# meteorologytoday/XLab-FFTBarotropic

Measured on AMD Instinct MI355X. Metric: RK4 steps/sec, 4096x4096 periodic grid, higher is better.
Workload: dtype f32; 1 GPU; 4096x4096 kuo2004 initial field, nu=6.5, L=600 km, dt=0.75 s, 4 RK stages/step, fused HIP path; parallelism=single

## Files before the change

xlab-fftbarotropic_amd/csrc/fb_col_full.h:

```cpp
#pragma once
#include "fb_kernels.h"

#define CF_THREADS 1024
#define CF_X1_CF 16384
#define CF_X2_STR 68
#define CF_X2_CF (16 * 16 * CF_X2_STR)
#define CF_GX_CF 2048
#define CF_LDS_CF (CF_X2_CF + 512 + CF_GX_CF)
#define CF_LDS_BYTES (CF_LDS_CF * 8)

struct FullArgs {
    const cf *Tin;
    const cf *Zbase;
    cf *Zcur, *Acc, *Zout;
    cf *W4;
    long fstride;
    int P;
    int ntiles;
    int ntiles_run;
    int nsub;
    int stage;
    float nu, dt;
    SpecCoef coef;
    const cf *tw256;
    const cf *tw4096;
    long sub_rows;
    float wscale;
};

FB_DEV void cf_xchg_waves(cf *lds, cf *v, int w, int lane)
{
#pragma unroll
    for (int r = 0; r < 16; ++r) lds_wr(&lds[(r * 16 + w) * 64 + lane], v[r]);
    lds_barrier();
#pragma unroll
    for (int r = 0; r < 16; ++r) v[r] = lds_rd(&lds[(w * 16 + r) * 64 + lane]);
    lds_barrier();
}

template <bool SYNC>
FB_DEV void cf_xchg_lanes(cf *lds, cf *v, int w, int l, int c)
{
    cf *reg = lds + w * (16 * CF_X2_STR);
#pragma unroll
    for (int r = 0; r < 16; ++r) lds_wr(&reg[r * CF_X2_STR + l * 4 + c], v[r]);
    __builtin_amdgcn_wave_barrier();
#pragma unroll
    for (int r = 0; r < 16; ++r) v[r] = lds_rd(&reg[l * CF_X2_STR + r * 4 + c]);
    if (SYNC) lds_barrier();
    else { asm volatile("s_waitcnt lgkmcnt(0)" ::: "memory"); __builtin_amdgcn_wave_barrier(); }
}

#define CF_FENCE() __builtin_amdgcn_sched_barrier(0)
FB_DEV cf cf_mul(cf a, cf b) { return cmul_split(a, b); }
FB_DEV cf cf_mulc(cf a, cf b) { return cmulc_split(a, b); }

template <int DIR> FB_DEV void cf_bfly16(cf *v)
{
    fft4<DIR>(v[0], v[4], v[8], v[12]);  CF_FENCE();
    fft4<DIR>(v[1], v[5], v[9], v[13]);  CF_FENCE();
    fft4<DIR>(v[2], v[6], v[10], v[14]); CF_FENCE();
    fft4<DIR>(v[3], v[7], v[11], v[15]); CF_FENCE();
    v[5]  = mul_w16<1, DIR, true>(v[5]);  v[6]  = mul_w16<2, DIR, true>(v[6]);  v[7]  = mul_w16<3, DIR, true>(v[7]);
    v[9]  = mul_w16<2, DIR, true>(v[9]);  v[10] = mul_w16<4, DIR, true>(v[10]); v[11] = mul_w16<6, DIR, true>(v[11]);
    v[13] = mul_w16<3, DIR, true>(v[13]); v[14] = mul_w16<6, DIR, true>(v[14]); v[15] = mul_w16<9, DIR, true>(v[15]);
    CF_FENCE();
    fft4<DIR>(v[0], v[1], v[2], v[3]);     CF_FENCE();
    fft4<DIR>(v[4], v[5], v[6], v[7]);     CF_FENCE();
    fft4<DIR>(v[8], v[9], v[10], v[11]);   CF_FENCE();
    fft4<DIR>(v[12], v[13], v[14], v[15]); CF_FENCE();
    cf t;
    t = v[1];  v[1]  = v[4];  v[4]  = t;
    t = v[2];  v[2]  = v[8];  v[8]  = t;
    t = v[3];  v[3]  = v[12]; v[12] = t;
    t = v[6];  v[6]  = v[9];  v[9]  = t;
    t = v[7];  v[7]  = v[13]; v[13] = t;
    t = v[11]; v[11] = v[14]; v[14] = t;
}

template <int DIR>
FB_DEV void cf_fft4096(cf *lds, const cf *tabA, const cf *tabB, cf (*v)[16], int w, int l, int c, int lane)
{
    if (DIR < 0) {
#pragma unroll
        for (int col = 0; col < 2; ++col) {
            cf_bfly16<-1>(v[col]);
#pragma unroll
            for (int k1 = 1; k1 < 16; ++k1) { v[col][k1] = cf_mul(v[col][k1], tabB[w * k1]); if ((k1 & 3) == 3) CF_FENCE(); }
            cf_xchg_waves(lds, v[col], w, lane);
            CF_FENCE();
        }
        const cf a = tabA[l * w];
#pragma unroll
        for (int col = 0; col < 2; ++col) {
            cf_bfly16<-1>(v[col]);
            v[col][0] = cf_mul(v[col][0], a);
#pragma unroll
            for (int k2 = 1; k2 < 16; ++k2) { v[col][k2] = cf_mul(v[col][k2], cf_mul(a, tabB[l * k2])); if ((k2 & 3) == 3) CF_FENCE(); }
            cf_xchg_lanes<false>(lds, v[col], w, l, c);
            CF_FENCE();
        }
#pragma unroll
        for (int col = 0; col < 2; ++col) { cf_bfly16<-1>(v[col]); CF_FENCE(); }
    } else {
#pragma unroll
        for (int col = 0; col < 2; ++col) {
            cf_bfly16<+1>(v[col]);
#pragma unroll
            for (int lr = 1; lr < 16; ++lr) { v[col][lr] = cf_mulc(v[col][lr], cf_mul(tabA[lr * w], tabB[lr * l])); if ((lr & 3) == 3) CF_FENCE(); }
            if (col == 0) cf_xchg_lanes<false>(lds, v[col], w, l, c);
            else cf_xchg_lanes<true>(lds, v[col], w, l, c);
            CF_FENCE();
        }
#pragma unroll
        for (int col = 0; col < 2; ++col) {
            cf_bfly16<+1>(v[col]);
#pragma unroll
            for (int wr = 1; wr < 16; ++wr) { v[col][wr] = cf_mulc(v[col][wr], tabB[wr * w]); if ((wr & 3) == 3) CF_FENCE(); }
            cf_xchg_waves(lds, v[col], w, lane);
            CF_FENCE();
        }
#pragma unroll
        for (int col = 0; col < 2; ++col) { cf_bfly16<+1>(v[col]); CF_FENCE(); }
    }
}

FB_DEV float4 cf_ld4(const void *ubase, unsigned voff) { return *reinterpret_cast<const float4 *>(static_cast<const char *>(ubase) + voff); }
FB_DEV void cf_st4(void *ubase, unsigned voff, float4 x) { *reinterpret_cast<float4 *>(static_cast<char *>(ubase) + voff) = x; }
FB_DEV void cf_st4_w4(void *ubase, unsigned voff, float4 x) { st4<true>(static_cast<char *>(ubase) + voff, x); }

template <int STAGE, int NSUB>
__global__ void __launch_bounds__(CF_THREADS) k_col_full(FullArgs a)
{
    extern __shared__ __attribute__((aligned(16))) unsigned char smem_raw[];
    cf *lds = reinterpret_cast<cf *>(smem_raw);
    cf *tabB = lds + CF_X2_CF, *tabA = tabB + 256;
    float *gxt = reinterpret_cast<float *>(tabA + 256);
    const int tid = threadIdx.x, lane = tid & 63, l = lane >> 2, c = lane & 3;
    const int w = __builtin_amdgcn_readfirstlane(tid >> 6);

    constexpr int nsub = NSUB;
    const int ntg = gridDim.x / nsub;
    const int k1 = NSUB == 1 ? 0 : blockIdx.x / ntg, bt = blockIdx.x - k1 * ntg;
    int tile = bt;
    if ((ntg & 7) == 0) tile = (bt & 7) * (ntg >> 3) + (bt >> 3);
    if (tile >= a.ntiles_run) return;

    const int ky0 = tile * 8 + 2 * c;
    const unsigned voff_m = (unsigned)((l * a.P + 2 * c) * (int)sizeof(cf));
    const size_t ubase_m = ((size_t)(k1 * a.sub_rows + 16 * w) * a.P + (size_t)tile * 8) * sizeof(cf);
    const size_t rstep = (size_t)256 * a.P * sizeof(cf);
    const unsigned voff_s = (unsigned)(lane * (int)sizeof(float4));
    const size_t ubase_s = ((((size_t)k1 * (a.ntiles + 1) + tile) * 16) * CF_THREADS + (size_t)w * 64) * sizeof(float4);
    const size_t sstep = (size_t)CF_THREADS * sizeof(float4);

    constexpr bool PRIME = STAGE == 4;
    cf v[2][16];
    {
        const char *src = reinterpret_cast<const char *>(a.Tin) + ubase_m;
        float4 tin[16];
        if (!PRIME) {
#pragma unroll
            for (int i = 0; i < 16; ++i) tin[i] = ld4<true>(src + i * rstep + voff_m);
        }
        float g4[4];
#pragma unroll
        for (int i = 0; i < 4; ++i) g4[i] = a.coef.gx[nsub * (tid + i * CF_THREADS) + k1];
        if (tid < 256) { tabB[tid] = a.tw256[tid]; tabA[tid] = a.tw4096[tid]; }
#pragma unroll
        for (int i = 0; i < 4; ++i) {
            const int ik = tid + i * CF_THREADS;
            gxt[((ik >> 4) & 15) + 16 * (ik & 15) + (ik & ~255)] = g4[i];
        }
        if (!PRIME) {
#pragma unroll
            for (int i = 0; i < 16; ++i) { v[0][i] = cf_make(tin[i].x, tin[i].y); v[1][i] = cf_make(tin[i].z, tin[i].w); }
        }
    }
    __syncthreads();
    if (!PRIME) cf_fft4096<-1>(lds, tabA, tabB, v, w, l, c, lane);

    const char *Z0 = reinterpret_cast<const char *>(a.Zbase) + ubase_s;
    char *ZC = reinterpret_cast<char *>(a.Zcur) + ubase_s, *AC = reinterpret_cast<char *>(a.Acc) + ubase_s,
         *ZO = reinterpret_cast<char *>(a.Zout) + ubase_s;
    const float gya = a.coef.gy[ky0], gyb = a.coef.gy[ky0 + 1];
    auto ky2_of = [](float g) { asm volatile("" : "+v"(g)); return (double)g * (double)g; };
    constexpr bool PRIME_ = STAGE == 4;
    const bool pada = PRIME_ && ky0 >= a.coef.hy, padb = PRIME_ && ky0 + 1 >= a.coef.hy;
    constexpr int stage = STAGE;
    const float nu = a.nu, dt = a.dt, hdt = (stage == 2) ? a.dt : a.dt / 2.0f;
    constexpr int DEPTH = STAGE == 0 ? 2 : 1;
#ifndef CF_REMAKE_ZC
#define CF_REMAKE_ZC 1
#endif
    constexpr bool REMAKE_ZC = CF_REMAKE_ZC && STAGE == 1;
    float4 q0[DEPTH], q1[DEPTH], q2[DEPTH];
    auto load_k3 = [&](int k3) {
        const int sl = k3 % DEPTH;
        q0[sl] = ld4<false>(Z0 + k3 * sstep + voff_s);
        if (stage != 0) q2[sl] = ld4<true>(AC + k3 * sstep + voff_s);
        if (stage != 0 && !REMAKE_ZC) q1[sl] = ld4<false>(ZC + k3 * sstep + voff_s);
    };
    if (!PRIME) {
#pragma unroll
        for (int k3 = 0; k3 < DEPTH; ++k3) load_k3(k3);
    }
#pragma unroll
    for (int k3 = 0; k3 < (PRIME ? 0 : 16); ++k3) {
        const int sl = k3 % DEPTH;
        const int ik2 = w + 256 * k3 + 16 * l, ikx = nsub * ik2 + k1;
        const float gx = gxt[l + 16 * w + 256 * k3];
        const double kx2 = (double)gx * (double)gx;
        const float lapa = (float)(-(kx2 + ky2_of(gya))), lapb = (float)(-(kx2 + ky2_of(gyb)));
        const float mska = coef_mask(a.coef, ikx, ky0), mskb = coef_mask(a.coef, ikx, ky0 + 1);
        const float4 z0 = q0[sl];
        float4 zc = z0;
        if (REMAKE_ZC) {
            const float4 ac = q2[sl];
            zc = make_float4(__builtin_fmaf(ac.x, hdt, z0.x), __builtin_fmaf(ac.y, hdt, z0.y), __builtin_fmaf(ac.z, hdt, z0.z), __builtin_fmaf(ac.w, hdt, z0.w));
        } else if (stage != 0) zc = q1[sl];
        float4 k;
        k.x = (v[0][k3].x + (zc.x * lapa) * nu) * mska; k.y = (v[0][k3].y + (zc.y * lapa) * nu) * mska;
        k.z = (v[1][k3].x + (zc.z * lapb) * nu) * mskb; k.w = (v[1][k3].y + (zc.w * lapb) * nu) * mskb;
        float4 acc, zn;
        if (stage == 0) {
            acc = k;
            zn = make_float4(__builtin_fmaf(k.x, hdt, z0.x), __builtin_fmaf(k.y, hdt, z0.y), __builtin_fmaf(k.z, hdt, z0.z), __builtin_fmaf(k.w, hdt, z0.w));
        } else if (stage < 3) {
            const float4 ac = q2[sl];
            acc = make_float4(ac.x + 2.0f * k.x, ac.y + 2.0f * k.y, ac.z + 2.0f * k.z, ac.w + 2.0f * k.w);
            zn = make_float4(z0.x + k.x * hdt, z0.y + k.y * hdt, z0.z + k.z * hdt, z0.w + k.w * hdt);
        } else {
            const float4 ac = q2[sl];
            acc = ac;
            zn = make_float4(z0.x + (ac.x + k.x) * dt / 6.0f, z0.y + (ac.y + k.y) * dt / 6.0f,
                             z0.z + (ac.z + k.z) * dt / 6.0f, z0.w + (ac.w + k.w) * dt / 6.0f);
        }
        v[0][k3] = cf_make(zn.x, zn.y); v[1][k3] = cf_make(zn.z, zn.w);
        if (k3 + DEPTH < 16) load_k3(k3 + DEPTH);
        if (stage < 3) { st4<true>(AC + k3 * sstep + voff_s, acc); cf_st4(ZC + k3 * sstep, voff_s, zn); }
        else cf_st4(ZO + k3 * sstep, voff_s, zn);
        CF_FENCE();
    }

    const char *ZN = PRIME ? Z0 : (stage < 3 ? ZC : ZO);
#pragma unroll 1
    for (int f = 0; f < 4; ++f) {
        if (f > 0 || PRIME) {
            const unsigned vs = (unsigned)launder((int)voff_s);
#pragma unroll
            for (int k3 = 0; k3 < 16; ++k3) {
                const float4 z = cf_ld4(ZN + k3 * sstep, vs);
                v[0][k3] = cf_make(z.x, z.y); v[1][k3] = cf_make(z.z, z.w);
            }
        }
        const bool psi = f >= 2, use_gx = (f == 0 || f == 3);
        const int lkx = launder(l);
#pragma unroll
        for (int k3 = 0; k3 < 16; ++k3) {
            cf za = v[0][k3], zb = v[1][k3];
            const float gx = gxt[16 * w + 256 * k3 + lkx];
            if (psi) {
                const double kx2 = (double)gx * (double)gx;
                const float lia = (nsub * (w + 256 * k3 + 16 * l) + k1 == 0 && ky0 == 0) ? 1.0f : (float)(-(kx2 + ky2_of(gya)));
                const float lib = (float)(-(kx2 + ky2_of(gyb)));
                za = pada ? cf_make(0.f, 0.f) : cf_make(za.x / lia, za.y / lia);
                zb = padb ? cf_make(0.f, 0.f) : cf_make(zb.x / lib, zb.y / lib);
            }
            const float ka = (use_gx ? gx : gya) * a.wscale, kb = (use_gx ? gx : gyb) * a.wscale;
            v[0][k3] = cf_make(-za.y * ka, za.x * ka);
            v[1][k3] = cf_make(-zb.y * kb, zb.x * kb);
            CF_FENCE();
        }
        cf_fft4096<+1>(lds, tabA, tabB, v, w, l, c, lane);
        char *dst = reinterpret_cast<char *>(a.W4) + (size_t)f * a.fstride * sizeof(cf) + ubase_m;
        const unsigned vm = (unsigned)launder((int)voff_m);
#pragma unroll
        for (int i = 0; i < 16; ++i)
            cf_st4_w4(dst + i * rstep, vm, make_float4(v[0][i].x, v[0][i].y, v[1][i].x, v[1][i].y));
    }
}

template <bool TO_FULL>
__global__ void __launch_bounds__(256) k_full_relayout(const cf *__restrict__ in, cf *__restrict__ out, int P, int N1, int N2, int ntiles, int nsub, int hy)
{
    const size_t total = (size_t)nsub * (ntiles + 1) * 16 * CF_THREADS * 2;
    for (size_t idx = (size_t)blockIdx.x * blockDim.x + threadIdx.x; idx < total; idx += (size_t)gridDim.x * blockDim.x) {
        const int col = (int)(idx & 1);
        const int tid = (int)((idx >> 1) & (CF_THREADS - 1));
        const int k3 = (int)((idx >> 11) & 15);
        const int st = (int)(idx >> 15);
        const int k1 = st / (ntiles + 1), tile = st - k1 * (ntiles + 1);
        const int w = tid >> 6, l = (tid >> 2) & 15, c = tid & 3;
        const int kx = nsub * (w + 16 * l + 256 * k3) + k1, ky = tile * 8 + 2 * c + col;
        const int cc = kx % N1, d = kx / N1;
        const size_t p3 = (size_t)(N2 * cc + d) * P + ky;
        if (ky >= hy) { if (TO_FULL) out[idx] = cf_make(0.f, 0.f); continue; }
        if (TO_FULL) out[idx] = in[p3]; else out[p3] = in[idx];
    }
}
```

xlab-fftbarotropic_amd/csrc/fftbaro.hip:

```cpp
#include <hip/hip_runtime.h>
#include <algorithm>
#include <cmath>
#include <cstdio>
#include <cstdlib>
#include <cstring>
#include <mutex>
#include <set>
#include <string>
#include <type_traits>
#include <utility>
#include <vector>

#include "../../include/fftbaro.h"
#include "fb_kernels.h"
#include "fb_keff.h"
#include "fb_azim.h"
#include "fb_spectra.h"
#include "fb_tracer.h"
#include "fb_particles.h"
#include "fb_tangent.h"
#include "fb_adjoint.h"
#include "fb_col_full.h"
#include "fb_row3.h"
#include "fb_row8.h"
// ... 724 lines not shown
        finish_groups(c);
        return FB_OK;
    }
    const size_t maxe = (size_t)c->nx * (P0 + 16 * (NC - 1));
    const int nbuf = xp != XP_COLS ? 9 : 1;
    cf *buf = nullptr;
    if (hipMalloc((void **)&buf, maxe * nbuf * sizeof(cf)) != hipSuccess) { hipGetLastError(); return FB_OK; }
    hipMemsetAsync(buf, 0, maxe * nbuf * sizeof(cf), c->stream);
    hipEvent_t e0, e1;
    hipEventCreate(&e0); hipEventCreate(&e1);
    auto probe = [&](int P) -> int {
        ColGroup G = c->grp[0]; G.ncols = P;
        if (xp == XP_COLS) return launch_col_strided<+1>(c, G, buf, 1, 0);
        FullArgs a; memset(&a, 0, sizeof(a));
        a.Tin = buf; a.W4 = buf + maxe; a.Zbase = buf + 5 * maxe; a.Zcur = buf + 6 * maxe; a.Acc = buf + 7 * maxe; a.Zout = buf + 8 * maxe;
        a.fstride = (long)c->nx * P; a.P = P; a.ntiles = (c->ny / 2) / 8;
        a.ntiles_run = a.ntiles; a.nsub = xp; a.stage = 1; a.nu = 0.f; a.dt = 0.f; a.coef = make_coef(c); a.tw256 = c->d_tw_256;
        a.tw4096 = xp == XP_FULL1 ? c->d_tw_big : c->d_tw_4096; a.sub_rows = 4096;
        return launch_full(c, a);
    };
    const bool verbose = c->tune_verbose;
    hipEventRecord(e0, c->stream);
    for (int it = 0; it < 400; ++it) {
        if (probe(P0) != FB_OK) break;
        if ((it & 7) == 7) {
            hipEventRecord(e1, c->stream); hipEventSynchronize(e1);
            float ms = 0.f;
            if (hipEventElapsedTime(&ms, e0, e1) != hipSuccess || ms > 30.f) break;
        }
    }
    float tbest[8]; for (int k = 0; k < NC; ++k) tbest[k] = 1e30f;
    for (int rep = 0; rep < 6; ++rep)
        for (int k = 0; k < NC; ++k) {
            hipEventRecord(e0, c->stream);
            const int rc = probe(P0 + 16 * k);
            hipEventRecord(e1, c->stream);
            hipEventSynchronize(e1);
            float ms = 0.f;
            if (rc == FB_OK && hipEventElapsedTime(&ms, e0, e1) == hipSuccess && ms < tbest[k]) tbest[k] = ms;
        }
    float best = 1e30f; int bestP = P0;
    for (int k = 0; k < NC; ++k) {
        if (verbose) fprintf(stderr, "fftbaro: pitch probe P=%d %.4f ms\n", P0 + 16 * k, tbest[k]);
        if (tbest[k] < best * 0.99f) { best = tbest[k]; bestP = P0 + 16 * k; }
    }
    if (verbose) fprintf(stderr, "fftbaro: pitch %d -> %d\n", P0, bestP);
    c->P = c->KA = c->katot = c->grp[0].ncols = bestP;
    finish_groups(c);
    hipEventDestroy(e0); hipEventDestroy(e1);
    hipFree(buf);
    hipGetLastError();
    return FB_OK;
}

static int ensure_scratch(fb_ctx *c)
{
    if (!c->d_scratch) {
        hipError_t e = hipMalloc((void **)&c->d_scratch, priv_elems(c) * sizeof(cf));
        if (e != hipSuccess) return fail(FB_ENOMEM, "scratch allocation failed");
    }
    return FB_OK;
}

static unsigned magic_div(int d) { return d > 0 ? (unsigned)((1ull << 32) / (unsigned)d) + 1u : 0u; }
static RowView view_single(const fb_ctx *c, const cf *base, long fstride)
{
    RowView v; memset(&v, 0, sizeof(v));
    v.a = v.b = v.f = base; v.fstrA = v.fstrB = v.fstrF = fstride; v.ka = v.ka0 = c->P; v.kb = 0; v.kf = 16; v.katot = 0x7fffffff;
    return v;
}
static RowView view_slab(const fb_ctx *c, const cf *const *bufs, int nfields)
{
    RowView v; memset(&v, 0, sizeof(v));
    v.a = bufs[0]; v.b = c->nact > 1 ? bufs[1] : bufs[0]; v.f = c->KF > 0 ? bufs[c->nact] : bufs[0];
    v.ka = c->KA; v.ka0 = c->grp[0].ncols; v.kb = c->nact > 1 ? c->grp[1].ncols : 0; v.kf = c->KF > 0 ? c->KF : 16;
    v.katot = c->katot;
    v.fstrA = (long)c->XL * v.ka0; v.fstrB = (long)c->XL * v.kb; v.fstrF = (long)c->XL * v.kf;
    v.sstrA = (long)nfields * v.fstrA; v.sstrB = (long)nfields * v.fstrB; v.sstrF = (long)nfields * v.fstrF;
    v.magA = magic_div(v.ka); v.magF = magic_div(v.kf);
    return v;
}
static RowArgs row_args_base(const fb_ctx *c)
{
    RowArgs a; memset(&a, 0, sizeof(a));
    a.x0 = 0; a.nx = c->XL; a.tw_bwd = c->d_tw_row_bwd; a.tw_fwd = c->d_tw_row_fwd; a.t_frozen = 1;
    return a;
}

static int r2c_private(fb_ctx *c, const float *d_real, cf *dst)
{
    RowArgs a = row_args_base(c); a.rin = d_real; a.T = view_single(c, dst, 0);
    int rc;
    if ((rc = launch_row<ROW_FWD>(c, a))) return rc;
    if ((rc = launch_col_strided<-1>(c, c->grp[0], dst, 1, 0))) return rc;
    return launch_col_block<-1>(c, c->grp[0], dst, 1, 0);
}

static int c2r_private(fb_ctx *c, cf *work, float *d_real, float scale)
{
    int rc;
    if ((rc = launch_col_block<+1>(c, c->grp[0], work, 1, 0))) return rc;
    if ((rc = launch_col_strided<+1>(c, c->grp[0], work, 1, 0))) return rc;
    RowArgs a = row_args_base(c); a.M = view_single(c, work, 0); a.rout = d_real; a.scale = scale;
    return launch_row<ROW_INV>(c, a);
}

static bool state_tm(const fb_ctx *c) { return c->N2 >= 32; }
static int state_convert(fb_ctx *c, const ColGroup &G, const cf *in, cf *out, bool to_tm)
{
    if (G.ncols == 0) return FB_OK;
    if (!state_tm(c)) { HIPCHK(hipMemcpyAsync(out, in, grp_elems(c, G) * sizeof(cf), hipMemcpyDeviceToDevice, c->stream)); return FB_OK; }
    const size_t total = grp_elems(c, G);
    return launch_n(c, to_tm ? k_state_relayout<true> : k_state_relayout<false>, total, in, out, c->nx, G.ncols, c->N2);
}

static int relayout(fb_ctx *c, const cf *in, cf *out, bool to_private)
{
    const size_t total = priv_elems(c);
    return launch_n(c, to_private ? k_spec_relayout<true> : k_spec_relayout<false>, total, in, out, c->nx, c->hy, c->P, c->N1, c->N2);
}

extern "C" int fb_r2c(fb_ctx *c, const float *d_in, float *d_out)
{
    if (!c || !d_in || !d_out) return fail(FB_EINVAL, "fb_r2c: NULL");
    NEED_SINGLE(c);
    int rc;
    if ((rc = ensure_scratch(c))) return rc;
    HIPCHK(hipMemsetAsync(c->d_scratch, 0, priv_elems(c) * sizeof(cf), c->stream));
    if ((rc = r2c_private(c, d_in, c->d_scratch))) return rc;
    return relayout(c, c->d_scratch, (cf *)d_out, false);
}

extern "C" int fb_c2r(fb_ctx *c, const float *d_in, float *d_out, int normalize)
{
    if (!c || !d_in || !d_out) return fail(FB_EINVAL, "fb_c2r: NULL");
    NEED_SINGLE(c);
    int rc;
    if ((rc = ensure_scratch(c))) return rc;
    if ((rc = relayout(c, (const cf *)d_in, c->d_scratch, true))) return rc;
    const float scale = normalize ? 1.0f / (float)((size_t)c->nx * c->ny) : 1.0f;
    return c2r_private(c, c->d_scratch, d_out, scale);
}

struct GroupBufs { cf *ZA, *ZB, *ACC, *w4_send, *w4_recv, *t_send, *t_recv; };

struct Beside { cf *c0[3], *c1[3], *acc[3]; };

struct fb_model {
    fb_ctx *c;
    float nu, dt;
    GroupBufs gb[3];
    bool phase_flow;
    XPass xpass;
    bool prescale;
    bool use_graph, warmed;
    hipGraphExec_t graph_exec;
    const float *graph_src; hipStream_t graph_stream;
    float *src;
    int *src_nz;
    cf *rec_work[3], *rec_send[3];
    float *keff_fields;
    void *keff_red; size_t keff_red_cap;
    float *azim_fields;
    void *azim_red; size_t azim_red_cap;
    float *pres_ref;
    unsigned char rec_work_nf[3], rec_send_nf[3];
    void *spec_red;
    int primed;
    Beside tr;
    float kappa;
    bool tracer;
    double *pt; int pt_n;
    float *pt_uv;
    Beside tg[FB_TANGENTS_MAX];
    int tg_n;
    cf *tg_j[3];
    double *tg_red;
    cf *ad_tape; int ad_depth, ad_fill;
    Beside ad;
    float *ad_real;
    bool adjoint;
};

#include "fb_transport.h"
struct fb_slab {
    fb_ctx *c;
    fb_model *m;
    fb_transport tp;
    bool connected, owns_streams;
    hipStream_t comp, comm;
    hipEvent_t ev_f[4], ev_r[8], ev_w4, ev_t, ev_tg[2], ev_rows_done, ev_fwd_done, ev_misc[2];
    int nfg, nch;
    int ncg;
    int step_ops;
};
#include "fb_entry.h"

static int model_create_impl(fb_model **out, fb_ctx *c, float nu, float dt, bool phase_flow)
{
    if (!out || !c) return fail(FB_EINVAL, "fb_model_create: NULL");
    *out = nullptr;
    fb_model *m = new fb_model();
    memset(m, 0, sizeof(*m));
    m->c = c; m->nu = nu; m->dt = dt; m->phase_flow = phase_flow;
    m->xpass = phase_flow ? XP_COLS : choose_xpass(c);
    m->prescale = m->xpass != XP_COLS && c->world == 1 && c->row == RK_ROWQ && !c->no_prescale;
    int rc = FB_OK;
    auto alloc0 = [&](cf **p, size_t elems) {
        if (rc || elems == 0) return;
        if (hipMalloc((void **)p, elems * sizeof(cf)) != hipSuccess) { rc = fail(FB_ENOMEM, "model allocation failed"); return; }
        if (hipMemsetAsync(*p, 0, elems * sizeof(cf), c->stream) != hipSuccess) rc = fail(FB_EHIP, "hipMemsetAsync failed");
    };
    for (int g = 0; g < c->ngroups; ++g) {
        const size_t n = grp_elems(c, c->grp[g]);
        GroupBufs &B = m->gb[g];
        alloc0(&B.ZA, n);
        if (g < c->nact) { alloc0(&B.ZB, n); alloc0(&B.ACC, n); }
        alloc0(&B.w4_send, 4 * n); alloc0(&B.t_send, n);
        if (c->world > 1) { alloc0(&B.w4_recv, 4 * n); alloc0(&B.t_recv, n); }
        else { B.w4_recv = B.w4_send; B.t_recv = B.t_send; }
    }
    if (rc) { fb_model_destroy(m); return rc; }
    *out = m;
    return FB_OK;
}

extern "C" int fb_model_create(fb_model **out, fb_ctx *c, float nu, float dt)
{
    if (c && c->world != 1) return fail(FB_EINVAL, "fb_model_create on a slab context: use fb_slab_create");
    return model_create_impl(out, c, nu, dt, false);
}

static int beside_stage(fb_model *m, fb_slab *s, int stage);
static void beside_step_done(fb_model *m);
static void beside_free_all(fb_model *m);

static void model_drop_graph(fb_model *m)
{
    if (m->graph_exec) { hipGraphExecDestroy(m->graph_exec); m->graph_exec = nullptr; }
}

static void state_replaced(fb_model *m)
{
    m->warmed = false;
    m->primed = 0;
    m->ad_fill = 0;
}

extern "C" int fb_model_destroy(fb_model *m)
{
    if (!m) return FB_OK;
    for (GroupBufs &B : m->gb) {
        if (B.w4_recv && B.w4_recv != B.w4_send) hipFree(B.w4_recv);
        if (B.t_recv && B.t_recv != B.t_send) hipFree(B.t_recv);
        cf *arr[] = {B.ZA, B.ZB, B.ACC, B.w4_send, B.t_send};
        for (cf *p : arr) if (p) hipFree(p);
    }
    model_drop_graph(m);
    if (m->src) hipFree(m->src);
    if (m->src_nz) hipFree(m->src_nz);
    for (auto p : m->rec_work) if (p) hipFree(p);
    for (auto p : m->rec_send) if (p) hipFree(p);
    if (m->keff_fields) hipFree(m->keff_fields);
    if (m->keff_red) hipFree(m->keff_red);
    if (m->azim_fields) hipFree(m->azim_fields);
    if (m->azim_red) hipFree(m->azim_red);
    if (m->pres_ref) hipFree(m->pres_ref);
    if (m->spec_red) hipFree(m->spec_red);
    beside_free_all(m);
    delete m;
    return FB_OK;
}

extern "C" int fb_model_info(fb_model *m, size_t *hbm, size_t *alg)
{
    if (int rc = enter(on_model("fb_model_info", m))) return rc;
    const fb_ctx *c = m->c;
    if (hbm) {
        size_t n = m->src ? (size_t)c->XL * c->ny * 4 : 0;
        for (int g = 0; g < c->ngroups; ++g) n += (c->world > 1 ? (g < c->nact ? 13 : 11) : 8) * grp_elems(c, c->grp[g]) * sizeof(cf);
        for (int g = 0; g < c->ngroups && m->tracer; ++g) n += (g < c->nact ? 3 : 1) * grp_elems(c, c->grp[g]) * sizeof(cf);
        if (m->pt_n) n += 6 * (size_t)m->pt_n * sizeof(double) + 2 * (size_t)c->nx * c->ny * sizeof(float);
        for (int g = 0; g < c->ngroups && m->tg_n; ++g)
            n += ((size_t)m->tg_n * (g < c->nact ? 3 : 1) + (g < c->nact ? 1 : 0)) * grp_elems(c, c->grp[g]) * sizeof(cf);
        *hbm = n;
    }
    if (alg) *alg = (size_t)320 * c->nx * c->ny;
    return FB_OK;
}

static int set_source(const Call &k, const float *d_src)
{
    if (int rc = enter(k)) return rc;
    fb_model *m = k.m;
    fb_ctx *c = m->c;
    const size_t n = (size_t)c->XL * c->ny * sizeof(float);
    if (!d_src) { if (m->src) { HIPCHK(hipStreamSynchronize(c->stream)); hipFree(m->src); m->src = nullptr; } return FB_OK; }
    if (!m->src_nz && hipMalloc((void **)&m->src_nz, (size_t)c->XL * sizeof(int)) != hipSuccess) { m->src_nz = nullptr; return fail(FB_ENOMEM, "source allocation failed"); }
    if (!m->src && hipMalloc((void **)&m->src, n) != hipSuccess) { m->src = nullptr; return fail(FB_ENOMEM, "source allocation failed"); }
    if (int rc = launch(c, k_src_row_flags, dim3(c->XL), dim3(256), 0, d_src, m->src_nz, c->ny)) return rc;
    const size_t half = (size_t)c->XL * c->ny / 2;
    switch (c->row) {
    case RK_ROWQ: return launch_n(c, k_rowq_permute_src, half, d_src, m->src, c->XL);
    case RK_ROWH_8192: return launch_n(c, k_rowh_permute_src<1>, half, d_src, m->src, c->XL);
    case RK_ROWH_16384: return launch_n(c, k_rowh_permute_src<2>, half, d_src, m->src, c->XL);
    default: HIPCHK(hipMemcpyAsync(m->src, d_src, n, hipMemcpyDeviceToDevice, c->stream)); return FB_OK;
    }
}
extern "C" int fb_model_set_source(fb_model *m, const float *d_src) { return set_source(on_model("fb_model_set_source", m), d_src); }
extern "C" int fb_slab_set_source_local(fb_slab *s, const float *d_rows) { return set_source(on_slab("fb_slab_set_source_local", s), d_rows); }

static MidArgs mid_args(fb_model *m, int g, int stage)
{
    fb_ctx *c = m->c;
    const ColGroup &G = c->grp[g];
    const GroupBufs &B = m->gb[g];
    MidArgs a;
    a.Tin = B.t_recv; a.Zbase = B.ZA; a.Zcur = B.ZB; a.Acc = B.ACC; a.Zout = B.ZA; a.W4 = B.w4_send;
    a.ct0 = 0; a.nct = stage < 0 ? G.ncols / 16 : G.nct_active;
    a.fstride = w4_fstride(c, G); a.rm = rowmap_w4(c, G); a.P = G.ncols; a.N1 = c->N1; a.N2 = c->N2; a.ky0 = G.ky0; a.stage = stage;
    a.nu = m->nu; a.dt = m->dt; a.coef = make_coef(c); a.tw_n = c->d_tw_n2; a.tw_big = c->d_tw_big;
    return a;
}

static int launch_col_full(fb_model *m, int stage)
{
    fb_ctx *c = m->c;
    const GroupBufs &B = m->gb[0];
    FullArgs a;
    a.Tin = B.t_recv; a.Zbase = B.ZA; a.Zcur = B.ZB; a.Acc = B.ACC; a.Zout = B.ZA; a.W4 = B.w4_send;
    a.fstride = (long)priv_elems(c); a.P = c->P; a.ntiles = (c->ny / 2) / 8; a.stage = stage; a.nu = m->nu; a.dt = m->dt;
    a.nsub = m->xpass; a.sub_rows = 4096;
    a.wscale = m->prescale ? 1.0f / (float)((size_t)c->nx * c->ny) : 1.0f;
    a.ntiles_run = c->grp[0].nct_active * 2 < a.ntiles ? c->grp[0].nct_active * 2 : a.ntiles;
    if (c->full_noskip) a.ntiles_run = a.ntiles;
    if (stage == 4) a.ntiles_run = a.ntiles + 1;
    a.coef = make_coef(c); a.tw256 = c->d_tw_256; a.tw4096 = m->xpass == XP_FULL1 ? c->d_tw_big : c->d_tw_4096;
    return launch_full(c, a);
}

static int full_import_state(fb_model *m, cf *spec3)
{
    fb_ctx *c = m->c;
    const int ntiles = (c->ny / 2) / 8;
    int rc;
    if ((rc = launch(c, k_full_relayout<true>, dim3(c->max_wg), dim3(256), 0, (const cf *)spec3, m->gb[0].ZA, c->P, c->N1, c->N2, ntiles, (int)m->xpass, c->hy)) ||
        (rc = launch_col_full(m, 4)))
        return rc;
    m->primed = 2;
    return FB_OK;
}

static int full_export_state(fb_model *m, cf *dst)
{
    fb_ctx *c = m->c;
    HIPCHK(hipMemsetAsync(dst, 0, priv_elems(c) * sizeof(cf), c->stream));
    const int ntiles = (c->ny / 2) / 8;
    return launch(c, k_full_relayout<false>, dim3(c->max_wg), dim3(256), 0, (const cf *)m->gb[0].ZA, dst, c->P, c->N1, c->N2, ntiles, (int)m->xpass, c->hy);
}

static int export_state(fb_model *m, int g, cf *dst)
{
    return m->xpass != XP_COLS ? full_export_state(m, dst) : state_convert(m->c, m->c->grp[g], m->gb[g].ZA, dst, false);
}

static int model_prime(fb_model *m)
{
    fb_ctx *c = m->c;
    int rc;
    for (int g = 0; g < c->ngroups; ++g) {
        const ColGroup &G = c->grp[g];
        if ((rc = launch_col_mid(c, mid_args(m, g, -1)))) return rc;
        if ((rc = launch_col_strided<+1>(c, G, m->gb[g].w4_send, 4, w4_fstride(c, G), rowmap_w4(c, G), G.nct_active, G.ncols / 16 - G.nct_active))) return rc;
    }
    m->primed = 1;
    return FB_OK;
}
static int model_col_bwd_active(fb_model *m, int f0 = 0, int f1 = 4, int g = 0)
{
    fb_ctx *c = m->c;
    const ColGroup &G = c->grp[g];
    return launch_col_strided<+1>(c, G, m->gb[g].w4_send + (size_t)f0 * w4_fstride(c, G), f1 - f0, w4_fstride(c, G), rowmap_w4(c, G), 0, G.nct_active);
}
static int launch_fused_row(fb_model *m, int x0, int nrows)
{
    fb_ctx *c = m->c;
    RowArgs a = row_args_base(c);
    if (c->world == 1) { a.M = view_single(c, m->gb[0].w4_recv, (long)priv_elems(c)); a.T = view_single(c, m->gb[0].t_send, 0); }
    else {
        const cf *w4[3] = {m->gb[0].w4_recv, m->gb[1].w4_recv, m->gb[2].w4_recv}, *ts[3] = {m->gb[0].t_send, m->gb[1].t_send, m->gb[2].t_send};
        a.M = view_slab(c, w4, 4); a.T = view_slab(c, ts, 1); a.t_frozen = 0;
    }
    a.src = m->src; a.src_nz = m->src_nz; a.scale = 1.0f / (float)((size_t)c->nx * c->ny); a.x0 = x0; a.nx = nrows; a.prescaled = m->prescale ? 1 : 0;
    return launch_row<ROW_FUSED>(c, a, m->xpass == XP_FULL2 ? RK_ROWH2 : c->row);
}
static int model_col_fwd(fb_model *m, int stage, int g = 0)
{
    fb_ctx *c = m->c;
    int rc;
    if ((rc = launch_col_strided<-1>(c, c->grp[g], m->gb[g].t_recv, 1, 0, rowmap_natural(), 0, c->grp[g].nct_active))) return rc;
    m->primed = 1;
    return launch_col_mid(c, mid_args(m, g, stage));
}

struct StepProf {
    std::vector<hipEvent_t> ev0[4], ev1[4];
    hipStream_t stream;
    int begin(int cls) { hipEvent_t a, b; if (hipEventCreate(&a) != hipSuccess || hipEventCreate(&b) != hipSuccess) return 1;
                         ev0[cls].push_back(a); ev1[cls].push_back(b); return hipEventRecord(a, stream) != hipSuccess; }
    int end(int cls) { return hipEventRecord(ev1[cls].back(), stream) != hipSuccess; }
};
#define PROF_BEGIN(cls) do { if (prof && prof->begin(cls)) return fail(FB_EHIP, "event record failed"); } while (0)
#define PROF_END(cls) do { if (prof && prof->end(cls)) return fail(FB_EHIP, "event record failed"); } while (0)

static int step_refusals(const Call &k, int nsteps)
{
    if (nsteps < 0) return refuse(k, "bad argument: nsteps < 0");
    if (int rc = enter(k, NEED_TRANSPORT)) return rc;
    const fb_model *m = k.m;
    if (m->ad_depth && nsteps > m->ad_depth - m->ad_fill)
        return refuse(k, "the adjoint's tape has room for " + std::to_string(m->ad_depth - m->ad_fill) + " more steps (fb_model_adjoint_record)");
    return FB_OK;
}

static int model_step_impl(fb_model *m, int nsteps, StepProf *prof)
{
    fb_ctx *c = m->c;
    int rc;
    if (nsteps == 0) return FB_OK;
    if (m->xpass != XP_COLS && !m->primed) return fail(FB_EINVAL, "fb_model_step: set the state first");
    if (!m->primed && (rc = model_prime(m))) return rc;
    if (m->primed == 1 && m->xpass == XP_COLS) { if ((rc = model_col_bwd_active(m))) return rc; m->primed = 2; }
    const ColGroup &G = c->grp[0];
    GroupBufs &B = m->gb[0];
    for (int s = 0; s < nsteps; ++s) {
        for (int k = 0; k < 4; ++k) {
            if ((rc = beside_stage(m, nullptr, k))) return rc;
            PROF_BEGIN(1);
            if ((rc = launch_fused_row(m, 0, c->XL))) return rc;
            PROF_END(1);
            if (m->xpass != XP_COLS) {
                PROF_BEGIN(3);
                if ((rc = launch_col_full(m, k))) return rc;
                PROF_END(3);
                continue;
            }
            PROF_BEGIN(2);
            if ((rc = launch_col_strided<-1>(c, G, B.t_recv, 1, 0, rowmap_natural(), 0, G.nct_active))) return rc;
            PROF_END(2);
            PROF_BEGIN(3);
            if ((rc = launch_col_mid(c, mid_args(m, 0, k)))) return rc;
            PROF_END(3);
            PROF_BEGIN(0);
            if ((rc = launch_col_strided<+1>(c, G, B.w4_send, 4, (long)priv_elems(c), rowmap_natural(), 0, G.nct_active))) return rc;
            PROF_END(0);
        }
        beside_step_done(m);
    }
    return FB_OK;
}

extern "C" int fb_model_use_graph(fb_model *m, int enable)
{
    if (int rc = enter(on_model("fb_model_use_graph", m))) return rc;
    m->use_graph = enable != 0;
    if (!m->use_graph) model_drop_graph(m);
    return FB_OK;
}

static int model_steps(fb_model *m, int nsteps)
{
    fb_ctx *c = m->c;
    if (!m->use_graph || c->world != 1 || c->stream == nullptr || nsteps < 2 || m->ad_depth) { if (nsteps > 0) m->warmed = true; return model_step_impl(m, nsteps, nullptr); }
    int rc;
    if (!m->warmed) { if ((rc = model_step_impl(m, 1, nullptr))) return rc; m->warmed = true; --nsteps; }
    if (m->graph_exec && (m->graph_src != m->src || m->graph_stream != c->stream)) model_drop_graph(m);
    if (!m->graph_exec) {
        hipGraph_t g = nullptr;
        HIPCHK(hipStreamBeginCapture(c->stream, hipStreamCaptureModeThreadLocal));
        rc = model_step_impl(m, 1, nullptr);
        hipError_t e = hipStreamEndCapture(c->stream, &g);
        if (rc) { if (g) hipGraphDestroy(g); return rc; }
        HIPCHK(e);
        e = hipGraphInstantiate(&m->graph_exec, g, nullptr, nullptr, 0);
        hipGraphDestroy(g);
        HIPCHK(e);
        m->graph_src = m->src; m->graph_stream = c->stream;
    }
    for (int s = 0; s < nsteps; ++s) HIPCHK(hipGraphLaunch(m->graph_exec, c->stream));
// ... 53 lines not shown
```

Before: 1208 steps/s.

## Skip fully dealiased x-bands and balance column-tile placement across XCDs

Adds a host-computed tile order that load-balances column tiles across eight groups (XCDs) using per-tile work weights, where the weights count bands lying entirely outside the dealiasing radius. Inside the fused column kernel, such frozen bands skip the RK update arithmetic and the Acc/Zcur loads and stores, and the subsequent FFT passes read them from the base state instead. Load prefetching is reordered to visit bands in an outside-in interleave with full 16-slot register buffers. This reduces memory traffic and balances work, at the cost of higher register pressure and extra control flow.

```diff
diff --git a/xlab-fftbarotropic_amd/csrc/fb_col_full.h b/xlab-fftbarotropic_amd/csrc/fb_col_full.h
--- a/xlab-fftbarotropic_amd/csrc/fb_col_full.h
+++ b/xlab-fftbarotropic_amd/csrc/fb_col_full.h
@@ -1,5 +1,6 @@
 #pragma once
 #include "fb_kernels.h"
+#include "fb_col_place.h"
 
 #define CF_THREADS 1024
 #define CF_X1_CF 16384
@@ -26,6 +27,8 @@
     const cf *tw4096;
     long sub_rows;
     float wscale;
+    const int *order;
+    int bandskip;
 };
 
 FB_DEV void cf_xchg_waves(cf *lds, cf *v, int w, int lane)
@@ -142,9 +145,13 @@
     constexpr int nsub = NSUB;
     const int ntg = gridDim.x / nsub;
     const int k1 = NSUB == 1 ? 0 : blockIdx.x / ntg, bt = blockIdx.x - k1 * ntg;
+    constexpr bool PRIME = STAGE == 4;
     int tile = bt;
     if ((ntg & 7) == 0) tile = (bt & 7) * (ntg >> 3) + (bt >> 3);
-    if (tile >= a.ntiles_run) return;
+    if (!PRIME && a.order) tile = a.order[bt];
+    if (tile < 0 || tile >= a.ntiles_run) return;
+    const unsigned fz = (!PRIME && a.bandskip) ? (unsigned)__builtin_amdgcn_readfirstlane((int)cf_frozen_bands(tile, k1, nsub, a.coef.gws_i)) : 0u;
+    auto frozen = [&](int k3) { if (PRIME) return false; unsigned f = fz; asm volatile("" : "+s"(f)); return (f >> k3 & 1u) != 0; };
 
     const int ky0 = tile * 8 + 2 * c;
     const unsigned voff_m = (unsigned)((l * a.P + 2 * c) * (int)sizeof(cf));
@@ -154,7 +161,6 @@
     const size_t ubase_s = ((((size_t)k1 * (a.ntiles + 1) + tile) * 16) * CF_THREADS + (size_t)w * 64) * sizeof(float4);
     const size_t sstep = (size_t)CF_THREADS * sizeof(float4);
 
-    constexpr bool PRIME = STAGE == 4;
     cf v[2][16];
     {
         const char *src = reinterpret_cast<const char *>(a.Tin) + ubase_m;
@@ -194,52 +200,79 @@
 #define CF_REMAKE_ZC 1
 #endif
     constexpr bool REMAKE_ZC = CF_REMAKE_ZC && STAGE == 1;
-    float4 q0[DEPTH], q1[DEPTH], q2[DEPTH];
+#define CF_AWAIT(q) asm volatile("" :: "v"((q).x), "v"((q).y))
+#define CF_AWAIT4(q) asm volatile("" :: "v"((q).x), "v"((q).y), "v"((q).z), "v"((q).w))
+    float4 q0[16], q1[16], q2[16];
     auto load_k3 = [&](int k3) {
-        const int sl = k3 % DEPTH;
-        q0[sl] = ld4<false>(Z0 + k3 * sstep + voff_s);
-        if (stage != 0) q2[sl] = ld4<true>(AC + k3 * sstep + voff_s);
-        if (stage != 0 && !REMAKE_ZC) q1[sl] = ld4<false>(ZC + k3 * sstep + voff_s);
+        const int sl = k3;
+        const unsigned vo = (unsigned)launder((int)voff_s);
+        q0[sl] = ld4<false>(Z0 + k3 * sstep + vo);
+        if (stage != 0) q2[sl] = ld4<true>(AC + k3 * sstep + vo);
+        if (stage != 0 && !REMAKE_ZC) q1[sl] = ld4<false>(ZC + k3 * sstep + vo);
     };
+    auto await_k3 = [&](int k3) {
+        CF_AWAIT4(q0[k3]);
+        if (stage != 0) CF_AWAIT4(q2[k3]);
+        if (stage != 0 && !REMAKE_ZC) CF_AWAIT4(q1[k3]);
+    };
+    auto band = [](int j) { return (j & 1) ? 15 - (j >> 1) : (j >> 1); };
     if (!PRIME) {
 #pragma unroll
-        for (int k3 = 0; k3 < DEPTH; ++k3) load_k3(k3);
-    }
-#pragma unroll
-    for (int k3 = 0; k3 < (PRIME ? 0 : 16); ++k3) {
-        const int sl = k3 % DEPTH;
-        const int ik2 = w + 256 * k3 + 16 * l, ikx = nsub * ik2 + k1;
-        const float gx = gxt[l + 16 * w + 256 * k3];
-        const double kx2 = (double)gx * (double)gx;
-        const float lapa = (float)(-(kx2 + ky2_of(gya))), lapb = (float)(-(kx2 + ky2_of(gyb)));
-        const float mska = coef_mask(a.coef, ikx, ky0), mskb = coef_mask(a.coef, ikx, ky0 + 1);
-        const float4 z0 = q0[sl];
-        float4 zc = z0;
-        if (REMAKE_ZC) {
-            const float4 ac = q2[sl];
-            zc = make_float4(__builtin_fmaf(ac.x, hdt, z0.x), __builtin_fmaf(ac.y, hdt, z0.y), __builtin_fmaf(ac.z, hdt, z0.z), __builtin_fmaf(ac.w, hdt, z0.w));
-        } else if (stage != 0) zc = q1[sl];
-        float4 k;
-        k.x = (v[0][k3].x + (zc.x * lapa) * nu) * mska; k.y = (v[0][k3].y + (zc.y * lapa) * nu) * mska;
-        k.z = (v[1][k3].x + (zc.z * lapb) * nu) * mskb; k.w = (v[1][k3].y + (zc.w * lapb) * nu) * mskb;
-        float4 acc, zn;
-        if (stage == 0) {
-            acc = k;
-            zn = make_float4(__builtin_fmaf(k.x, hdt, z0.x), __builtin_fmaf(k.y, hdt, z0.y), __builtin_fmaf(k.z, hdt, z0.z), __builtin_fmaf(k.w, hdt, z0.w));
-        } else if (stage < 3) {
-            const float4 ac = q2[sl];
-            acc = make_float4(ac.x + 2.0f * k.x, ac.y + 2.0f * k.y, ac.z + 2.0f * k.z, ac.w + 2.0f * k.w);
-            zn = make_float4(z0.x + k.x * hdt, z0.y + k.y * hdt, z0.z + k.z * hdt, z0.w + k.w * hdt);
-        } else {
-            const float4 ac = q2[sl];
-            acc = ac;
-            zn = make_float4(z0.x + (ac.x + k.x) * dt / 6.0f, z0.y + (ac.y + k.y) * dt / 6.0f,
-                             z0.z + (ac.z + k.z) * dt / 6.0f, z0.w + (ac.w + k.w) * dt / 6.0f);
-        }
-        v[0][k3] = cf_make(zn.x, zn.y); v[1][k3] = cf_make(zn.z, zn.w);
-        if (k3 + DEPTH < 16) load_k3(k3 + DEPTH);
-        if (stage < 3) { st4<true>(AC + k3 * sstep + voff_s, acc); cf_st4(ZC + k3 * sstep, voff_s, zn); }
-        else cf_st4(ZO + k3 * sstep, voff_s, zn);
+        for (int k3 = 0; k3 < 16; ++k3)
+            if (frozen(k3)) {
+                const float4 z = ld4<false>(Z0 + k3 * sstep + voff_s);
+                v[0][k3] = cf_make(z.x, z.y); v[1][k3] = cf_make(z.z, z.w);
+            }
+#pragma unroll
+        for (int j = 0; j < DEPTH; ++j)
+            if (!frozen(band(j))) load_k3(band(j));
+#pragma unroll
+        for (int k3 = 0; k3 < 16; ++k3) { CF_AWAIT(v[0][k3]); CF_AWAIT(v[1][k3]); }
+    }
+#pragma unroll
+    for (int j = 0; j < (PRIME ? 0 : 16); ++j) {
+        const int k3 = band(j);
+        if (!frozen(k3)) {
+            const int sl = k3;
+            if (j >= DEPTH && frozen(band(j >= DEPTH ? j - DEPTH : j))) {
+                load_k3(k3);
+                await_k3(k3);
+            }
+            await_k3(k3);
+            const int ik2 = w + 256 * k3 + 16 * l, ikx = nsub * ik2 + k1;
+            const float gx = gxt[l + 16 * w + 256 * k3];
+            const double kx2 = (double)gx * (double)gx;
+            const float lapa = (float)(-(kx2 + ky2_of(gya))), lapb = (float)(-(kx2 + ky2_of(gyb)));
+            const float mska = coef_mask(a.coef, ikx, ky0), mskb = coef_mask(a.coef, ikx, ky0 + 1);
+            const float4 z0 = q0[sl];
+            float4 zc = z0;
+            if (REMAKE_ZC) {
+                const float4 ac = q2[sl];
+                zc = make_float4(__builtin_fmaf(ac.x, hdt, z0.x), __builtin_fmaf(ac.y, hdt, z0.y), __builtin_fmaf(ac.z, hdt, z0.z), __builtin_fmaf(ac.w, hdt, z0.w));
+            } else if (stage != 0) zc = q1[sl];
+            float4 k;
+            k.x = (v[0][k3].x + (zc.x * lapa) * nu) * mska; k.y = (v[0][k3].y + (zc.y * lapa) * nu) * mska;
+            k.z = (v[1][k3].x + (zc.z * lapb) * nu) * mskb; k.w = (v[1][k3].y + (zc.w * lapb) * nu) * mskb;
+            float4 acc, zn;
+            if (stage == 0) {
+                acc = k;
+                zn = make_float4(__builtin_fmaf(k.x, hdt, z0.x), __builtin_fmaf(k.y, hdt, z0.y), __builtin_fmaf(k.z, hdt, z0.z), __builtin_fmaf(k.w, hdt, z0.w));
+            } else if (stage < 3) {
+                const float4 ac = q2[sl];
+                acc = make_float4(ac.x + 2.0f * k.x, ac.y + 2.0f * k.y, ac.z + 2.0f * k.z, ac.w + 2.0f * k.w);
+                zn = make_float4(z0.x + k.x * hdt, z0.y + k.y * hdt, z0.z + k.z * hdt, z0.w + k.w * hdt);
+            } else {
+                const float4 ac = q2[sl];
+                acc = ac;
+                zn = make_float4(z0.x + (ac.x + k.x) * dt / 6.0f, z0.y + (ac.y + k.y) * dt / 6.0f,
+                                 z0.z + (ac.z + k.z) * dt / 6.0f, z0.w + (ac.w + k.w) * dt / 6.0f);
+            }
+            v[0][k3] = cf_make(zn.x, zn.y); v[1][k3] = cf_make(zn.z, zn.w);
+            if (j + DEPTH < 16 && !frozen(band(j + DEPTH < 16 ? j + DEPTH : j))) load_k3(band(j + DEPTH < 16 ? j + DEPTH : j));
+            const unsigned vo = (unsigned)launder((int)voff_s);
+            if (stage < 3) { st4<true>(AC + k3 * sstep + vo, acc); cf_st4(ZC + k3 * sstep, vo, zn); }
+            else cf_st4(ZO + k3 * sstep, vo, zn);
+        }
         CF_FENCE();
     }
 
@@ -250,7 +283,7 @@
             const unsigned vs = (unsigned)launder((int)voff_s);
 #pragma unroll
             for (int k3 = 0; k3 < 16; ++k3) {
-                const float4 z = cf_ld4(ZN + k3 * sstep, vs);
+                const float4 z = cf_ld4((frozen(k3) ? Z0 : ZN) + k3 * sstep, vs);
                 v[0][k3] = cf_make(z.x, z.y); v[1][k3] = cf_make(z.z, z.w);
             }
         }
diff --git a/xlab-fftbarotropic_amd/csrc/fb_col_place.h b/xlab-fftbarotropic_amd/csrc/fb_col_place.h
--- /dev/null
+++ b/xlab-fftbarotropic_amd/csrc/fb_col_place.h
@@ -0,0 +1,88 @@
+#pragma once
+#include <algorithm>
+#include <vector>
+
+#if defined(__HIPCC__)
+#define CF_HD __host__ __device__
+#else
+#define CF_HD
+#endif
+
+CF_HD inline unsigned cf_frozen_bands(int tile, int k1, int nsub, int gws_i)
+{
+    const int nx = nsub * 4096, t8 = 8 * tile;
+    unsigned fz = 0;
+    for (int k3 = 0; k3 < 16; ++k3) {
+        const int lo = nsub * 256 * k3 + k1, hi = nsub * (256 * k3 + 255) + k1;
+        const int m = k3 < 8 ? lo : nx - hi;
+        if (m * m + t8 * t8 >= gws_i) fz |= 1u << k3;
+    }
+    return fz;
+}
+
+inline int cf_tile_weight(int tile, int nsub, int gws_i)
+{
+    int w = 0;
+    for (int k1 = 0; k1 < nsub; ++k1) {
+        const unsigned fz = cf_frozen_bands(tile, k1, nsub, gws_i);
+        int frozen = 0;
+        for (int k3 = 0; k3 < 16; ++k3) frozen += (fz >> k3) & 1;
+        w += 8 * 16 + 4 * (16 - frozen) + frozen;
+    }
+    return w;
+}
+
+inline std::vector<int> cf_tile_order(int ntiles, int ntiles_run, int nsub, int gws_i)
+{
+    std::vector<int> order;
+    if (ntiles <= 0 || ntiles % 16 != 0 || ntiles_run < 0 || ntiles_run > ntiles) return order;
+    const int np = (ntiles_run + 1) / 2, cap = ntiles / 16;
+    std::vector<int> wp(np), idx(np);
+    for (int p = 0; p < np; ++p) {
+        wp[p] = cf_tile_weight(2 * p, nsub, gws_i) + (2 * p + 1 < ntiles_run ? cf_tile_weight(2 * p + 1, nsub, gws_i) : 0);
+        idx[p] = p;
+    }
+    std::stable_sort(idx.begin(), idx.end(), [&](int a, int b) { return wp[a] > wp[b]; });
+    std::vector<int> on[8];
+    long W[8] = {0, 0, 0, 0, 0, 0, 0, 0};
+    for (int p : idx) {
+        int x = -1;
+        for (int y = 0; y < 8; ++y)
+            if ((int)on[y].size() < cap && (x < 0 || W[y] < W[x])) x = y;
+        on[x].push_back(p); W[x] += wp[p];
+    }
+    for (int it = 0; it < 100000; ++it) {
+        int h = 0;
+        for (int y = 1; y < 8; ++y) if (W[y] > W[h]) h = y;
+        long best = W[h];
+        int bx = -1, bi = -1, bj = -1;
+        for (int x = 0; x < 8; ++x) {
+            if (x == h) continue;
+            for (int i = 0; i < (int)on[h].size(); ++i) {
+                const long wa = wp[on[h][i]];
+                if ((int)on[x].size() < cap) {
+                    const long r = std::max(W[h] - wa, W[x] + wa);
+                    if (r < best) { best = r; bx = x; bi = i; bj = -1; }
+                }
+                for (int j = 0; j < (int)on[x].size(); ++j) {
+                    const long d = wa - wp[on[x][j]];
+                    if (d <= 0) continue;
+                    const long r = std::max(W[h] - d, W[x] + d);
+                    if (r < best) { best = r; bx = x; bi = i; bj = j; }
+                }
+            }
+        }
+        if (bx < 0) break;
+        const int pa = on[h][bi];
+        if (bj < 0) { on[h].erase(on[h].begin() + bi); on[bx].push_back(pa); W[h] -= wp[pa]; W[bx] += wp[pa]; }
+        else { const int pb = on[bx][bj]; on[h][bi] = pb; on[bx][bj] = pa; W[h] -= wp[pa] - wp[pb]; W[bx] += wp[pa] - wp[pb]; }
+    }
+    order.assign(ntiles, -1);
+    for (int x = 0; x < 8; ++x)
+        for (int j = 0; j < (int)on[x].size(); ++j) {
+            const int p = on[x][j];
+            order[(2 * j) * 8 + x] = 2 * p;
+            if (2 * p + 1 < ntiles_run) order[(2 * j + 1) * 8 + x] = 2 * p + 1;
+        }
+    return order;
+}
diff --git a/xlab-fftbarotropic_amd/csrc/fftbaro.hip b/xlab-fftbarotropic_amd/csrc/fftbaro.hip
--- a/xlab-fftbarotropic_amd/csrc/fftbaro.hip
+++ b/xlab-fftbarotropic_amd/csrc/fftbaro.hip
@@ -900,6 +900,7 @@
     GroupBufs gb[3];
     bool phase_flow;
     XPass xpass;
+    int *cf_order;
     bool prescale;
     bool use_graph, warmed;
     hipGraphExec_t graph_exec;
@@ -944,6 +945,17 @@
 };
 #include "fb_entry.h"
 
+static int full_ntiles_run(const fb_ctx *c)
+{
+    const int ntiles = (c->ny / 2) / 8;
+    if (c->full_noskip) return ntiles;
+    return c->grp[0].nct_active * 2 < ntiles ? c->grp[0].nct_active * 2 : ntiles;
+}
+
+#ifndef CF_PLACE
+#define CF_PLACE 1
+#endif
+
 static int model_create_impl(fb_model **out, fb_ctx *c, float nu, float dt, bool phase_flow)
 {
     if (!out || !c) return fail(FB_EINVAL, "fb_model_create: NULL");
@@ -968,6 +980,14 @@
         if (c->world > 1) { alloc0(&B.w4_recv, 4 * n); alloc0(&B.t_recv, n); }
         else { B.w4_recv = B.w4_send; B.t_recv = B.t_send; }
     }
+    if (!rc && m->xpass != XP_COLS && !c->full_noskip && CF_PLACE && (int)m->xpass * ((c->ny / 2) / 8) > c->max_wg / 8) {
+        const SpecCoef coef = make_coef(c);
+        const std::vector<int> order = cf_tile_order((c->ny / 2) / 8, full_ntiles_run(c), (int)m->xpass, coef.gws_i);
+        if (!order.empty()) {
+            if (hipMalloc((void **)&m->cf_order, order.size() * sizeof(int)) != hipSuccess) { m->cf_order = nullptr; rc = fail(FB_ENOMEM, "model allocation failed"); }
+            else if (hipMemcpy(m->cf_order, order.data(), order.size() * sizeof(int), hipMemcpyHostToDevice) != hipSuccess) rc = fail(FB_EHIP, "hipMemcpy failed");
+        }
+    }
     if (rc) { fb_model_destroy(m); return rc; }
     *out = m;
     return FB_OK;
@@ -1005,6 +1025,7 @@
         for (cf *p : arr) if (p) hipFree(p);
     }
     model_drop_graph(m);
+    if (m->cf_order) hipFree(m->cf_order);
     if (m->src) hipFree(m->src);
     if (m->src_nz) hipFree(m->src_nz);
     for (auto p : m->rec_work) if (p) hipFree(p);
@@ -1080,9 +1101,8 @@
     a.fstride = (long)priv_elems(c); a.P = c->P; a.ntiles = (c->ny / 2) / 8; a.stage = stage; a.nu = m->nu; a.dt = m->dt;
     a.nsub = m->xpass; a.sub_rows = 4096;
     a.wscale = m->prescale ? 1.0f / (float)((size_t)c->nx * c->ny) : 1.0f;
-    a.ntiles_run = c->grp[0].nct_active * 2 < a.ntiles ? c->grp[0].nct_active * 2 : a.ntiles;
-    if (c->full_noskip) a.ntiles_run = a.ntiles;
-    if (stage == 4) a.ntiles_run = a.ntiles + 1;
+    a.ntiles_run = stage == 4 ? a.ntiles + 1 : full_ntiles_run(c);
+    a.order = stage == 4 ? nullptr : m->cf_order; a.bandskip = (stage != 4 && m->cf_order) ? 1 : 0;
     a.coef = make_coef(c); a.tw256 = c->d_tw_256; a.tw4096 = m->xpass == XP_FULL1 ? c->d_tw_big : c->d_tw_4096;
     return launch_full(c, a);
 }
diff --git a/xlab-fftbarotropic_amd/host/col_place_check.cpp b/xlab-fftbarotropic_amd/host/col_place_check.cpp
--- /dev/null
+++ b/xlab-fftbarotropic_amd/host/col_place_check.cpp
@@ -0,0 +1,18 @@
+#include <cstdio>
+#include <cstdlib>
+
+#include "../csrc/fb_col_place.h"
+
+int main(int argc, char **argv)
+{
+    if (argc != 5) { fprintf(stderr, "usage: NSUB NTILES NTILES_RUN GWS_I\n"); return 2; }
+    const int nsub = atoi(argv[1]), ntiles = atoi(argv[2]), run = atoi(argv[3]), gws_i = atoi(argv[4]);
+    if (nsub < 1 || nsub > 2 || ntiles < 1 || ntiles > 512 || run < 0 || run > ntiles) { fprintf(stderr, "bad argument\n"); return 2; }
+    for (int t = 0; t < run; ++t)
+        for (int k1 = 0; k1 < nsub; ++k1) printf("bands %d %d %x\n", t, k1, cf_frozen_bands(t, k1, nsub, gws_i));
+    const std::vector<int> order = cf_tile_order(ntiles, run, nsub, gws_i);
+    printf("order");
+    for (int t : order) printf(" %d", t);
+    printf("\n");
+    return 0;
+}
```

Result: no change. 1215 steps/s (median of 3 runs) (+0.6%).
